# bensonlzl/spaced-kmer-sketching

Hardware: AMD Instinct MI355X
Metric: k-mers hashed/s + genome-pairs ANI/s at 1/2/4/8 MI355X; % HBM roofline (higher is better)
Workload: dtype u64; 1 GPU; config3: 1x3 Gb multi-contig genome per GPU, spaced seed w=31/k=21 (mask seed 0), FracMinHash 1/1000; builds_in_flight=3, genome_bytes=3000000024, windows_per_genome=2999036400, sketch_size=2998764, parallelism=genome-sharded x1

## Files before the change

### spaced-kmer-sketching_amd/csrc/build.cpp

```cpp
#include <cstdlib>
#include <numeric>
#include <utility>

#include "build_internal.hpp"

using namespace sks;

BuildKnobs sks::read_build_knobs() {
  static const bool scan_static = getenv("SKS_SCAN_STATIC") != nullptr;
  BuildKnobs k;
  k.no_fused_bottom = getenv("SKS_NO_FUSED_BOTTOM") != nullptr;
  k.no_fast_bottom = getenv("SKS_NO_FAST_BOTTOM") != nullptr;
  k.no_frac_fused = getenv("SKS_NO_FRAC_FUSED") != nullptr;
  k.scan_static = scan_static;
  return k;
}

int sks::validate_build(const char* fn, sks_ctx* c, const uint8_t* d_seq, uint64_t n_bytes, const uint64_t* seg_off,
                        uint32_t n_seg, int window, const uint64_t mask[2], const sks_policy* policy) {
  const std::string f(fn);
  if (!c || !mask || !policy || (!seg_off && n_seg)) return sks::fail(SKS_E_ARG, f + ": null argument");
  if (window < 1 || window > 64)
    return sks::fail(SKS_E_ARG, f + ": window must be in [1, 64] (MAX_KMER_LENGTH)");
  if (policy->kind != SKS_FRAC_MOD && policy->kind != SKS_BOTTOM_S)
// ... 29 lines not shown
  *out = {{}, arena.ptr(o_extra), arena.ptr(o_cnt), arena.ptr(o_cnt) + 2 * (m + 1)};
  sks::ScanParams& p = out->p;
  p.seq = d_seq;
  p.seg_begin = arena.ptr(o_beg);
  p.seg_end = arena.ptr(o_end);
  p.tile_prefix = arena.ptr(o_tiles);
  p.n_seg = g.m();
  p.n_tiles = g.n_tiles();
  p.w = S.w;
  p.mask_lo = S.mask_lo;
  p.mask_hi = S.mask_hi;
  p.kconst = S.kconst;
  p.low_mask = S.dt.low_mask;
  p.high_mask = S.dt.rot > 32 ? (uint32_t)((1ull << (S.dt.rot - 32)) - 1) : 0u;
  p.dinv = S.dt.dinv;
  p.dlim = S.dt.lim;
  p.seg_thresh = arena.ptr(list_mode ? o_cap : o_thr);
  p.out_key = reinterpret_cast<uint64_t*>(c->rec[0].ptr);
  p.seg_out_off = arena.ptr(o_off);
  p.seg_out_cap = arena.ptr(o_cap);
  p.seg_count = reinterpret_cast<unsigned long long*>(out->counters);
  p.seg_windows = reinterpret_cast<unsigned long long*>(out->counters + m + 1);
  if (list_mode) return SKS_OK;
  p.out_val = reinterpret_cast<uint64_t*>(c->rec[1].ptr);
  p.out_hi = reinterpret_cast<uint64_t*>(c->rec[2].ptr);
  p.tile_queue = S.knobs.scan_static ? nullptr : reinterpret_cast<unsigned long long*>(arena.ptr(o_queue));
  return SKS_OK;
}

namespace {

constexpr int kFastFallback = -1;
constexpr int kFastPostFallback = -2;

int make_single_set(const BuildState& S, uint64_t slots, SetPtr* one) {
  const uint64_t mask[2] = {S.mask_lo, S.mask_hi};
  return make_sketch_set(S.c->device, 1, S.w, mask, S.pol, {0}, {0}, {}, &slots, S.c->stream, MetaUpload::kNone, one);
}

template <class Post>
int run_single(const BuildState& S, const ScanMeta& meta, int mode, Post post, uint64_t h[6]) {
  sks_ctx* c = S.c;
  hipStream_t st = c->stream;
  hipError_t e = hipEventRecord(c->ev_s0, st);
  if (e == hipSuccess) e = sks::launch_scan(meta.p, mode, S.pol.flavour, false, c->device, st, c->grid_override);
  if (e == hipSuccess) e = hipEventRecord(c->ev_s1, st);
  if (e == hipSuccess) e = post();
// ... 43 lines not shown
  }, h));
  const uint64_t survivors = h[0], windows = h[2], size = h[4];
  if (survivors > cap || size == ~0ull || size == sks::kBottomOverflow || size > slots) return kFastFallback;
  scan_timings(c, seg.n_tiles(), survivors, tm);
  finish_single(S, tm, windows, size, one, out);
  return SKS_OK;
}

int build_frac_single(BuildState& S, const uint8_t* d_seq, const uint64_t* seg_off, uint64_t cap, int log_b,
                      sks_timings& tm, sks_sketch_set** out, uint64_t* survivors_out, uint64_t* windows_out) {
  sks_ctx* c = S.c;
  hipStream_t st = c->stream;
  const uint32_t bucket_cap = c->frac_bucket_cap
                                  ? std::min<uint32_t>(c->frac_bucket_cap, sks::frac_bucket_capacity())
                                  : sks::frac_bucket_capacity();
  const uint64_t slots = std::max<uint64_t>(cap, 1);
  SKS_HIP(c->rec[0].reserve(slots * sizeof(uint64_t)));
  SKS_HIP(c->buf[0].reserve(((uint64_t)bucket_cap << log_b) * sizeof(uint64_t)));
  SKS_HIP(c->fstate.reserve(sks::frac_state_bytes()));
  if (!c->fstate_clean) SKS_HIP(hipMemsetAsync(c->fstate.ptr, 0, sks::frac_state_bytes(), st));
  c->fstate_clean = false;
  ScanSegs seg;
  seg.push(seg_off[0], seg_off[1], ~0ull, cap);
  ScanMeta meta;
  SKS_TRY(scan_meta(S, d_seq, seg, false, {}, 2, &meta));
  SetPtr one;
  SKS_TRY(make_single_set(S, slots, &one));
  uint64_t h[6] = {0, 0, 0, 0, 0, 0};
  const int rc = run_single(S, meta, sks::kModeFrac, [&] {
    const hipError_t e = sks::launch_frac_fused(
        reinterpret_cast<uint64_t*>(c->rec[0].ptr), meta.counters, meta.p.seg_out_cap, slots, S.key_bits, S.runs,
        (uint32_t)log_b, bucket_cap, col(c, 0), reinterpret_cast<uint32_t*>(c->fstate.ptr), one->d_data(),
        one->d_sizes(), one->d_starts(), meta.results, st);
    if (e == hipSuccess) c->fstate_clean = true;
    return e;
  }, h);
  if (rc != SKS_OK) {
    c->fstate_clean = false;
    return rc;
  }
  const uint64_t survivors = h[0], windows = h[2], size = h[4], status = h[5];
  scan_timings(c, seg.n_tiles(), survivors, tm);
  *survivors_out = survivors;
  if (survivors > cap || size > survivors) return kFastFallback;
  if (status != 0) {
    *windows_out = windows;
    return kFastPostFallback;
  }
  finish_single(S, tm, windows, size, one, out);
  c->last_path = SKS_BUILD_PATH_FUSED;
  return SKS_OK;
}

struct Passes {
  std::vector<SegPlan> plan;
  std::vector<uint64_t> windows;
// ... 172 lines not shown
```

### spaced-kmer-sketching_amd/csrc/post.hip

```cpp
#include <hip/hip_runtime.h>

#include <algorithm>
#include <cstdio>
#include <cstring>
#include <rocprim/rocprim.hpp>
#include <rocprim/block/block_radix_sort.hpp>

#include "code_objects.hpp"
#include "device_mem.hpp"
#include "post.hpp"
#include "sks_hash.hpp"
#include "wave_prims.hpp"

namespace sks {

hipError_t Scratch::reserve(size_t n) {
  if (n <= bytes) return hipSuccess;
  const size_t grown = bytes + bytes / 2;
  if (ptr) {
    if (owner) {
      cache_release_after(ptr, bytes, *owner);
    } else {
      (void)hipDeviceSynchronize();
      (void)hipFree(ptr);
// ... 52 lines not shown
    return hipSuccess;
  }
  size_t need = 0;
  hipError_t e;
  if constexpr (PAIRS)
    e = rocprim::segmented_radix_sort_pairs(nullptr, need, keys_in, keys_out, vals_in, vals_out,
                                            (unsigned)total, (unsigned)n_seg, d_off, d_off + 1, 0,
                                            end_bit, s);
  else
    e = rocprim::segmented_radix_sort_keys(nullptr, need, keys_in, keys_out, (unsigned)total,
                                           (unsigned)n_seg, d_off, d_off + 1, 0, end_bit, s);
  if (e != hipSuccess) return e;
  if ((e = tmp.reserve(need)) != hipSuccess) return e;
  need = tmp.bytes;
  if constexpr (PAIRS)
    return rocprim::segmented_radix_sort_pairs(tmp.ptr, need, keys_in, keys_out, vals_in, vals_out,
                                               (unsigned)total, (unsigned)n_seg, d_off, d_off + 1,
                                               0, end_bit, s);
  else
    return rocprim::segmented_radix_sort_keys(tmp.ptr, need, keys_in, keys_out, (unsigned)total,
                                              (unsigned)n_seg, d_off, d_off + 1, 0, end_bit, s);
}

__device__ __forceinline__ uint64_t runs_pack(uint64_t x, const BitRuns& r) {
  x &= r.mask;
#pragma unroll
  for (int i = 0; i < 6; ++i) {
    const uint64_t mv = r.mv[i];
    if (mv) {
      const uint64_t t = x & mv;
      x = (x ^ t) | (t >> (1 << i));
    }
  }
  return x;
}

__device__ __forceinline__ uint64_t runs_expand(uint64_t x, const BitRuns& r) {
  const int width = __popcll(r.mask);
  if (width < 64) x &= (1ull << width) - 1;
#pragma unroll
  for (int i = 5; i >= 0; --i) {
    const uint64_t mv = r.mv[i];
    if (mv) x = (x & ~mv) | ((x << (1 << i)) & mv);
  }
  return x & r.mask;
}

template <bool PACK>
__global__ void k_compact(const uint64_t* __restrict__ src, uint64_t* __restrict__ dst,
                          const uint64_t* __restrict__ src_off, const uint64_t* __restrict__ dst_off,
                          const BitRuns runs, int tag_shift) {
  const uint32_t g = blockIdx.y;
  const uint64_t len = dst_off[g + 1] - dst_off[g];
  const uint64_t so = src_off[g], d0 = dst_off[g];
  const uint64_t tag = tag_shift >= 0 ? (uint64_t)g << tag_shift : 0;
  for (uint64_t i = (uint64_t)blockIdx.x * kB + threadIdx.x; i < len; i += (uint64_t)gridDim.x * kB)
    dst[d0 + i] = (PACK ? runs_pack(src[so + i], runs) : src[so + i]) | tag;
}

__global__ void k_bits_expand(uint64_t* __restrict__ keys, uint64_t n, const BitRuns runs) {
  for (uint64_t i = (uint64_t)blockIdx.x * kB + threadIdx.x; i < n; i += (uint64_t)gridDim.x * kB)
    keys[i] = runs_expand(keys[i], runs);
}

__global__ void k_flags(const uint64_t* __restrict__ keys, const uint64_t* __restrict__ keys2,
                        const uint64_t* __restrict__ off, uint32_t* __restrict__ flag) {
  const uint32_t g = blockIdx.y;
  const uint64_t b = off[g], e = off[g + 1];
  for (uint64_t i = b + (uint64_t)blockIdx.x * kB + threadIdx.x; i < e; i += (uint64_t)gridDim.x * kB) {
    bool first = (i == b) || keys[i] != keys[i - 1] || (keys2 && keys2[i] != keys2[i - 1]);
// ... 493 lines not shown
    lt_m |= (lt ? 1u : 0u) << j;
    eq_m |= (eq ? 1u : 0u) << j;
  }
  uint32_t eq_rank = block_excl_scan<kSelWaves>((uint32_t)__builtin_popcount(eq_m), wsum);
  __syncthreads();
  uint32_t keep_m = lt_m;
#pragma unroll
  for (uint32_t j = 0; j < ITEMS; ++j)
    if ((eq_m >> j) & 1u) keep_m |= (eq_rank++ < sel.kk ? 1u : 0u) << j;
  uint32_t pos = block_excl_scan<kSelWaves>((uint32_t)__builtin_popcount(keep_m), wsum);
  __syncthreads();
  uint64_t* skept = reinterpret_cast<uint64_t*>(smem);
#pragma unroll
  for (uint32_t j = 0; j < ITEMS; ++j)
    if ((keep_m >> j) & 1u) skept[pos++] = k[j];
  __syncthreads();
  for (uint32_t i = tid; i < (uint32_t)lim; i += kSelB) dst[i] = runs_expand(skept[i], runs);
}

constexpr int kFracB = 256;
constexpr int kFracWaves = kFracB / 64;
constexpr uint32_t kFracItems = 16;
constexpr uint32_t kFracCap = kFracB * kFracItems;
constexpr int kFracPartB = 1024;
constexpr uint32_t kFracPartTile = 1u << 14;
constexpr int kFracSubLog = 11;
constexpr uint32_t kFracSub = 1u << kFracSubLog;
constexpr uint32_t kFracSubPer = kFracSub / kFracB;
constexpr uint32_t kFracSubMax = 32;
constexpr uint32_t kFracMaxLogB = 14;
constexpr uint32_t kFracStateCounts = 1u << kFracMaxLogB;
constexpr uint32_t kFracStateStatus = 2u << kFracMaxLogB;

__global__ __launch_bounds__(kFracPartB) void k_frac_partition(const uint64_t* __restrict__ rec,
                                                               const uint64_t* __restrict__ seg_count,
                                                               const uint64_t* __restrict__ seg_cap,
                                                               const BitRuns runs, int shift, uint32_t n_buckets,
                                                               uint32_t bucket_cap, uint64_t* __restrict__ regions,
                                                               uint32_t* __restrict__ state) {
  extern __shared__ uint32_t s_cur[];
  const uint64_t n = seg_count[0];
  if (n > seg_cap[0]) return;
  const uint64_t rows = (n + kFracPartB - 1) / kFracPartB;
  const uint64_t share = (rows + gridDim.x - 1) / gridDim.x * kFracPartB;
  const uint64_t lo = min((uint64_t)blockIdx.x * share, n), hi = min(lo + share, n);
  if (lo >= hi) return;
  auto bucket_of = [&](uint64_t key) {
    const uint64_t top = shift < 64 ? key >> shift : 0ull;
    return (uint32_t)min(top, (uint64_t)(n_buckets - 1));
  };
  for (uint32_t b = threadIdx.x; b < n_buckets; b += kFracPartB) s_cur[b] = 0;
  __syncthreads();
#pragma unroll 4
  for (uint64_t i = lo + threadIdx.x; i < hi; i += kFracPartB) atomicAdd(&s_cur[bucket_of(runs_pack(rec[i], runs))], 1u);
  __syncthreads();
  for (uint32_t b = threadIdx.x; b < n_buckets; b += kFracPartB) {
    const uint32_t c = s_cur[b];
    if (c) s_cur[b] = atomicAdd(&state[b], c);
  }
  __syncthreads();
  bool over = false;
#pragma unroll 4
  for (uint64_t i = lo + threadIdx.x; i < hi; i += kFracPartB) {
    const uint64_t key = runs_pack(rec[i], runs);
    const uint32_t b = bucket_of(key);
    const uint32_t slot = atomicAdd(&s_cur[b], 1u);
    if (slot < bucket_cap) regions[(uint64_t)b * bucket_cap + slot] = key;
    else over = true;
  }
  if (over) atomicOr(&state[kFracStateStatus], (uint32_t)kFracStatusBucket);
}

template <uint32_t ITEMS>
__device__ __forceinline__ void frac_sort_body(uint64_t* __restrict__ reg, uint32_t n, uint32_t b,
                                               uint32_t* __restrict__ state, const BitRuns& runs, int shift,
                                               uint64_t* skeys, uint32_t* sbin, uint32_t* wsum, uint32_t* wmax) {
  const int tid = threadIdx.x;
  uint64_t k[ITEMS];
#pragma unroll
  for (uint32_t j = 0; j < ITEMS; ++j) {
    const uint32_t i = j * kFracB + tid;
    k[j] = i < n ? reg[i] : ~0ull;
  }
  const uint64_t low = shift >= 64 ? ~0ull : (1ull << shift) - 1;
  const int sub_shift = shift > kFracSubLog ? shift - kFracSubLog : 0;
  auto sub_of = [&](uint64_t key) { return (uint32_t)min((key & low) >> sub_shift, (uint64_t)(kFracSub - 1)); };
#pragma unroll
  for (uint32_t j = 0; j < ITEMS; ++j)
    if (j * kFracB + tid < n) atomicAdd(&sbin[sub_of(k[j])], 1u);
  __syncthreads();
  uint32_t cb[kFracSubPer], sum = 0, mx = 0;
#pragma unroll
  for (uint32_t q = 0; q < kFracSubPer; ++q) {
    cb[q] = sbin[tid * kFracSubPer + q];
// ... 48 lines not shown
  }
  __syncthreads();
  const uint64_t before = tid ? skeys[tid * ITEMS - 1] : 0ull;
  uint32_t first_m = 0;
#pragma unroll
  for (uint32_t j = 0; j < ITEMS; ++j) {
    const uint32_t i = tid * ITEMS + j;
    k[j] = skeys[i];
    const bool first = i < n && (i == 0 || k[j] != (j ? k[j - 1] : before));
    first_m |= (first ? 1u : 0u) << j;
  }
  uint32_t distinct;
  uint32_t pos = block_excl_scan<kFracWaves>((uint32_t)__builtin_popcount(first_m), wsum, &distinct);
  __syncthreads();
#pragma unroll
  for (uint32_t j = 0; j < ITEMS; ++j)
    if ((first_m >> j) & 1u) skeys[pos++] = k[j];
  __syncthreads();
  for (uint32_t i = tid; i < distinct; i += kFracB) reg[i] = runs_expand(skeys[i], runs);
  if (tid == 0) state[kFracStateCounts + b] = distinct;
}

__global__ __launch_bounds__(kFracB) void k_frac_sort_unique(uint64_t* __restrict__ regions,
                                                             uint32_t* __restrict__ state, const BitRuns runs,
                                                             int shift, uint32_t bucket_cap) {
  __shared__ uint64_t skeys[kFracCap];
  __shared__ uint32_t sbin[kFracSub];
  __shared__ uint32_t wsum[kFracWaves], wmax[kFracWaves];
  __shared__ uint32_t s_n;
  const uint32_t b = blockIdx.x;
  const int tid = threadIdx.x;
  uint32_t* counts = state + kFracStateCounts;
  if (tid == 0) {
    s_n = state[b];
    state[b] = 0;
  }
#pragma unroll
  for (uint32_t q = 0; q < kFracSubPer; ++q) sbin[tid * kFracSubPer + q] = 0;
  __syncthreads();
  const uint32_t n = s_n;
  if (n == 0 || n > bucket_cap) {
    if (tid == 0) {
      counts[b] = 0;
      if (n) atomicOr(&state[kFracStateStatus], (uint32_t)kFracStatusBucket);
    }
    return;
  }
  uint64_t* reg = regions + (uint64_t)b * bucket_cap;
  if (n <= 4 * kFracB) frac_sort_body<4>(reg, n, b, state, runs, shift, skeys, sbin, wsum, wmax);
  else if (n <= 8 * kFracB) frac_sort_body<8>(reg, n, b, state, runs, shift, skeys, sbin, wsum, wmax);
  else frac_sort_body<kFracItems>(reg, n, b, state, runs, shift, skeys, sbin, wsum, wmax);
}

__global__ __launch_bounds__(kFracB) void k_frac_gather(const uint64_t* __restrict__ regions,
                                                        uint32_t* __restrict__ state, uint32_t n_buckets,
                                                        uint32_t bucket_cap, uint64_t out_cap,
                                                        uint64_t* __restrict__ out, uint32_t* __restrict__ set_sizes,
// ... 45 lines not shown
                          uint64_t* vals_out, uint64_t total, const std::vector<uint64_t>& host_off,
                          const uint64_t* d_off, int end_bit, Scratch& tmp, hipStream_t s) {
  return sort_impl<true>(keys_in, keys_out, vals_in, vals_out, total, host_off, d_off, end_bit,
                         tmp, s);
}

hipError_t compact_regions(const uint64_t* src, uint64_t* dst, const uint64_t* d_src_off,
                           const uint64_t* d_dst_off, uint32_t n_seg, uint64_t max_len,
                           hipStream_t s, const BitRuns* pack, int tag_shift) {
  if (n_seg == 0 || max_len == 0) return hipSuccess;
  if (pack && pack->n)
    hipLaunchKernelGGL(k_compact<true>, dim3(grid_for(max_len), n_seg), dim3(kB), 0, s, src, dst,
                       d_src_off, d_dst_off, *pack, tag_shift);
  else
    hipLaunchKernelGGL(k_compact<false>, dim3(grid_for(max_len), n_seg), dim3(kB), 0, s, src, dst,
                       d_src_off, d_dst_off, BitRuns{}, tag_shift);
  return hipGetLastError();
}

hipError_t launch_seg_ids(uint64_t* out, const uint64_t* d_off, uint32_t n_seg, uint64_t max_len, hipStream_t s) {
  if (n_seg == 0 || max_len == 0) return hipSuccess;
  hipLaunchKernelGGL(k_seg_ids, dim3(grid_for(max_len), n_seg), dim3(kB), 0, s, out, d_off);
  return hipGetLastError();
}

BitRuns bit_runs(uint64_t mask) {
  BitRuns r;
  for (int b = 0; b < 64; ++b)
    if (((mask >> b) & 1) && (b == 0 || !((mask >> (b - 1)) & 1))) ++r.n;
  r.mask = mask;
  uint64_t m = mask, mk = ~m << 1;
  for (int i = 0; i < 6; ++i) {
    uint64_t mp = mk ^ (mk << 1);
    for (int sh = 2; sh < 64; sh <<= 1) mp ^= mp << sh;
    const uint64_t mv = mp & m;
    r.mv[i] = mv;
    m = (m ^ mv) | (mv >> (1 << i));
    mk &= ~mp;
  }
  return r;
}

hipError_t launch_bits_expand(uint64_t* keys, uint64_t n, const BitRuns& runs, hipStream_t s) {
  if (n == 0 || runs.n == 0) return hipSuccess;
  hipLaunchKernelGGL(k_bits_expand, dim3(grid_for(n)), dim3(kB), 0, s, keys, n, runs);
  return hipGetLastError();
}

hipError_t seg_unique_scan(const uint64_t* keys, const uint64_t* keys2, uint64_t total,
                           uint64_t max_len, const uint64_t* d_off, uint32_t n_seg, uint32_t* d_flag,
                           uint64_t* d_pos, uint64_t* d_uniq, Scratch& tmp, hipStream_t s) {
  if (n_seg == 0) return hipSuccess;
  hipError_t e;
  if (total) {
    hipLaunchKernelGGL(k_flags, dim3(grid_for(std::min<uint64_t>(max_len, 1ull << 24)), n_seg),
                       dim3(kB), 0, s, keys, keys2, d_off, d_flag);
    if ((e = hipGetLastError()) != hipSuccess) return e;
  }
  if ((e = hipMemsetAsync(d_flag + total, 0, sizeof(uint32_t), s)) != hipSuccess) return e;
  size_t need = 0;
  e = rocprim::exclusive_scan(nullptr, need, d_flag, d_pos, (uint64_t)0, (size_t)(total + 1),
                              rocprim::plus<uint64_t>(), s);
  if (e != hipSuccess) return e;
// ... 153 lines not shown
                               uint64_t* set_starts) {
  if (n_seg == 0) return hipSuccess;
  if (max_cnt > kFuseCap) return hipErrorInvalidValue;
  auto go = [&](auto kernel, size_t lds) -> hipError_t {
    const hipError_t a = hipFuncSetAttribute(reinterpret_cast<const void*>(kernel),
                                             hipFuncAttributeMaxDynamicSharedMemorySize, (int)lds);
    if (a != hipSuccess) return a;
    hipLaunchKernelGGL(kernel, dim3(n_seg), dim3(kSelB), lds, s, rec, d_src_off, d_cnt, d_retry_ok,
                       d_dst_off, s_param, key_bits, runs, kconst, out, d_res, d_cap, set_sizes, set_starts);
    return hipGetLastError();
  };
  if (max_cnt <= kSelB * 8)
    return flavour == 0 ? go(k_bottom_fused<0, 8>, fuse_lds<8>()) : go(k_bottom_fused<1, 8>, fuse_lds<8>());
  if (max_cnt <= kSelB * 12)
    return flavour == 0 ? go(k_bottom_fused<0, 12>, fuse_lds<12>())
                        : go(k_bottom_fused<1, 12>, fuse_lds<12>());
  return flavour == 0 ? go(k_bottom_fused<0, 16>, fuse_lds<16>()) : go(k_bottom_fused<1, 16>, fuse_lds<16>());
}

uint32_t frac_bucket_capacity() { return kFracCap; }
uint32_t frac_max_log_buckets() { return kFracMaxLogB; }
size_t frac_state_bytes() { return (size_t)(kFracStateStatus + 2) * sizeof(uint32_t); }

hipError_t launch_frac_fused(const uint64_t* rec, const uint64_t* d_cnt, const uint64_t* d_cap, uint64_t cap,
                             int key_bits, const BitRuns& runs, uint32_t log_b, uint32_t bucket_cap,
                             uint64_t* regions, uint32_t* state, uint64_t* out, uint32_t* set_sizes,
                             uint64_t* set_starts, uint64_t* d_res, hipStream_t s) {
  if (log_b > kFracMaxLogB || bucket_cap == 0 || bucket_cap > kFracCap || key_bits < 1 || key_bits > 64)
    return hipErrorInvalidValue;
  const uint32_t n_buckets = 1u << log_b;
  const int shift = key_bits > (int)log_b ? key_bits - (int)log_b : 0;
  const uint64_t tiles = (std::max<uint64_t>(cap, 1) + kFracPartTile - 1) / kFracPartTile;
  hipLaunchKernelGGL(k_frac_partition, dim3((unsigned)std::min<uint64_t>(tiles, 256)), dim3(kFracPartB),
                     n_buckets * sizeof(uint32_t), s, rec, d_cnt, d_cap, runs, shift, n_buckets, bucket_cap, regions,
                     state);
  hipLaunchKernelGGL(k_frac_sort_unique, dim3(n_buckets), dim3(kFracB), 0, s, regions, state, runs, shift,
                     bucket_cap);
  hipLaunchKernelGGL(k_frac_gather, dim3(n_buckets), dim3(kFracB), 0, s, regions, state, n_buckets, bucket_cap,
                     cap, out, set_sizes, set_starts, d_res);
  return hipGetLastError();
}

hipError_t launch_iota(uint64_t* out, uint64_t n, hipStream_t s) {
  if (n == 0) return hipSuccess;
  hipLaunchKernelGGL(k_iota, dim3(grid_for(n)), dim3(kB), 0, s, out, n);
  return hipGetLastError();
}

hipError_t launch_gather(const uint64_t* src, const uint64_t* idx, uint64_t n, uint64_t* out,
                         hipStream_t s) {
  if (n == 0) return hipSuccess;
  hipLaunchKernelGGL(k_gather, dim3(grid_for(n)), dim3(kB), 0, s, src, idx, n, out);
  return hipGetLastError();
}

hipError_t launch_interleave(const uint64_t* lo, const uint64_t* hi, uint64_t n, uint64_t* out,
                             hipStream_t s) {
  if (n == 0) return hipSuccess;
  hipLaunchKernelGGL(k_interleave, dim3(grid_for(n)), dim3(kB), 0, s, lo, hi, n, out);
  return hipGetLastError();
// ... 6 lines not shown
```

### spaced-kmer-sketching_amd/csrc/post.hpp

```cpp
#pragma once
#include <hip/hip_runtime.h>

#include <cstdint>
#include <vector>

#include "build_plan.hpp"
#include "device_mem.hpp"

namespace sks {

hipError_t seg_sort_keys(const uint64_t* keys_in, uint64_t* keys_out, uint64_t total,
                         const std::vector<uint64_t>& host_off, const uint64_t* d_off,
                         int end_bit, Scratch& tmp, hipStream_t s);
hipError_t seg_sort_pairs(const uint64_t* keys_in, uint64_t* keys_out, const uint64_t* vals_in,
                          uint64_t* vals_out, uint64_t total, const std::vector<uint64_t>& host_off,
                          const uint64_t* d_off, int end_bit, Scratch& tmp, hipStream_t s);

struct BitRuns {
  uint32_t n = 0;
  uint64_t mask = 0;
  uint64_t mv[6] = {0, 0, 0, 0, 0, 0};
};
BitRuns bit_runs(uint64_t mask);
hipError_t launch_bits_expand(uint64_t* keys, uint64_t n, const BitRuns& runs, hipStream_t s);
constexpr uint64_t kBottomOverflow = ~1ull;
uint32_t bottom_fused_capacity();
hipError_t launch_bottom_fused(uint64_t* rec, const uint64_t* d_src_off, const uint64_t* d_cnt,
                               const uint64_t* d_retry_ok, const uint64_t* d_dst_off,
                               uint32_t n_seg, uint64_t max_cnt, uint64_t s_param, int key_bits,
                               const BitRuns& runs, uint64_t kconst, int flavour, uint64_t* out,
                               uint64_t* d_res, hipStream_t s, const uint64_t* d_cap = nullptr,
                               uint32_t* set_sizes = nullptr, uint64_t* set_starts = nullptr);

constexpr uint64_t kFracStatusBucket = 1;
constexpr uint64_t kFracStatusCrowd = 2;
uint32_t frac_bucket_capacity();
uint32_t frac_max_log_buckets();
size_t frac_state_bytes();
hipError_t launch_frac_fused(const uint64_t* rec, const uint64_t* d_cnt, const uint64_t* d_cap, uint64_t cap,
                             int key_bits, const BitRuns& runs, uint32_t log_b, uint32_t bucket_cap,
                             uint64_t* regions, uint32_t* state, uint64_t* out, uint32_t* set_sizes,
                             uint64_t* set_starts, uint64_t* d_res, hipStream_t s);

hipError_t compact_regions(const uint64_t* src, uint64_t* dst, const uint64_t* d_src_off,
                           const uint64_t* d_dst_off, uint32_t n_seg, uint64_t max_len,
                           hipStream_t s, const BitRuns* pack = nullptr, int tag_shift = -1);
hipError_t launch_seg_ids(uint64_t* out, const uint64_t* d_off, uint32_t n_seg, uint64_t max_len, hipStream_t s);

hipError_t seg_unique_scan(const uint64_t* keys, const uint64_t* keys2, uint64_t total,
                           uint64_t max_len, const uint64_t* d_off, uint32_t n_seg, uint32_t* d_flag,
                           uint64_t* d_pos, uint64_t* d_uniq, Scratch& tmp, hipStream_t s);
hipError_t sort_unique_u64(const uint64_t* in, uint64_t n, uint64_t* out, uint64_t* n_out,
                           Scratch& tmp, hipStream_t s);
hipError_t sort_unique_u128(const uint64_t* in, uint64_t n, uint64_t* out, uint64_t* n_out,
                            Scratch& tmp, hipStream_t s);
hipError_t seg_unique_scatter(const uint64_t* vals, const uint64_t* vals2, uint64_t total,
                              uint64_t max_len, const uint64_t* d_off, uint32_t n_seg,
                              const uint32_t* d_flag,
                              const uint64_t* d_pos, const uint64_t* d_limit,
                              const uint64_t* d_dst_off, uint64_t* out, uint64_t* out2,
                              hipStream_t s, const BitRuns* expand = nullptr, uint64_t keep = ~0ull,
                              uint64_t keep2 = ~0ull);

hipError_t launch_synth(uint8_t* out, uint64_t n, uint64_t seed, uint64_t mut_seed,
                        uint64_t mut_thresh, uint64_t pos_offset, hipStream_t s);
// ... 19 lines not shown
```

### spaced-kmer-sketching_amd/csrc/scan.hip

```cpp
#include <hip/hip_runtime.h>

#include <cstdlib>

#include <cstdint>
#include <type_traits>

#include "code_objects.hpp"
#include "scan.hpp"
#include "sks_hash.hpp"

namespace sks {

namespace {

constexpr int kBlock = 256;
constexpr int kWPT = 16;
constexpr int kTile = kBlock * kWPT;
constexpr int kHaloWords = 4;
constexpr int kWords = kBlock + kHaloWords;
constexpr int kLoadVecs = (kWords * 16 + 16) / 16;
constexpr int kQCap = 2048;
#ifndef SKS_SCAN_QCAP
#define SKS_SCAN_QCAP 512
#endif
template <int MODE>
constexpr int qcap() { return MODE == kModeList ? kQCap : SKS_SCAN_QCAP; }
// ... 154 lines not shown

__device__ __forceinline__ uint32_t rev_pairs(uint32_t x) {
  uint32_t r = __builtin_bitreverse32(x);
  return ((r >> 1) & 0x55555555u) | ((r & 0x55555555u) << 1);
}


__device__ __forceinline__ unsigned long long wave_aggregated_inc(unsigned long long* counter) {
  const uint64_t act = __ballot(true);
  const uint32_t rank = __builtin_amdgcn_mbcnt_hi((uint32_t)(act >> 32),
                                                  __builtin_amdgcn_mbcnt_lo((uint32_t)act, 0u));
  unsigned long long base = 0;
  if (rank == 0) base = atomicAdd(counter, (unsigned long long)__popcll(act));
  const uint32_t lo = __builtin_amdgcn_readfirstlane((uint32_t)base);
  const uint32_t hi = __builtin_amdgcn_readfirstlane((uint32_t)(base >> 32));
  return (((unsigned long long)hi << 32) | lo) + rank;
}

template <int MODE>
struct Queue {
  uint64_t key[qcap<MODE>()];
  uint64_t val[MODE == kModeBottom ? qcap<MODE>() : 1];
  uint32_t n;
  unsigned long long base;
  unsigned long long wins;
};

template <int MODE>
__device__ __forceinline__ void emit(const ScanParams& p, Queue<MODE>& q, uint32_t seg,
                                     uint64_t key, uint64_t val) {
  uint32_t slot = atomicAdd(&q.n, 1u);
  if (slot < (uint32_t)qcap<MODE>()) {
    q.key[slot] = key;
    if constexpr (MODE == kModeBottom) q.val[slot] = val;
  } else {
    unsigned long long g = wave_aggregated_inc(&p.seg_count[seg]);
    if (g < p.seg_out_cap[seg]) {
      uint64_t o = p.seg_out_off[seg] + g;
      p.out_key[o] = key;
      if constexpr (MODE == kModeBottom) p.out_val[o] = val;
    }
  }
}

template <int MODE>
__device__ __forceinline__ void flush(const ScanParams& p, Queue<MODE>& q, uint32_t seg) {
  __syncthreads();
  if (threadIdx.x == 0 && q.wins) atomicAdd(&p.seg_windows[seg], q.wins);
  constexpr uint32_t cap = qcap<MODE>();
  uint32_t n = q.n < cap ? q.n : cap;
  if (n) {
    if (threadIdx.x == 0) q.base = atomicAdd(&p.seg_count[seg], (unsigned long long)n);
    __syncthreads();
    uint64_t base = q.base;
    uint64_t cap = p.seg_out_cap[seg];
    uint64_t off = p.seg_out_off[seg];
    for (uint32_t i = threadIdx.x; i < n; i += kBlock) {
      if (base + i < cap) {
        p.out_key[off + base + i] = q.key[i];
        if constexpr (MODE == kModeBottom) p.out_val[off + base + i] = q.val[i];
      }
    }
  }
  __syncthreads();
  if (threadIdx.x == 0) {
    q.n = 0;
    q.wins = 0;
  }
  __syncthreads();
}

__device__ __forceinline__ void add_windows(unsigned long long& wins, uint32_t cnt) {
  uint32_t v = cnt;
#pragma unroll
  for (int o = 32; o > 0; o >>= 1) v += __shfl_xor(v, o, 64);
  if ((threadIdx.x & 63) == 0 && v) atomicAdd(&wins, (unsigned long long)v);
}

template <int FLAVOUR>
__device__ __forceinline__ uint64_t fmh_narrow(const ScanParams& p, uint64_t c) {
  uint64_t h;
  if constexpr (FLAVOUR == 0) {
    h = hash_mix(c + kGolden32);
    h = hash_mix(h + kGolden32);
    h = hash_mix(h + (128 + kGolden32));
  } else {
    h = hash_bitset128<1>(c, 0);
  }
  return h ^ p.kconst;
}
// ... 37 lines not shown
__global__ __launch_bounds__(kBlock, (min_waves<MODE, PRE, FMIN>())) void scan_kernel(ScanParams p) {
  __shared__ uint32_t s_raw[kLoadVecs * 4];
  __shared__ uint32_t s_be[kWords + 2 + kBeOff];
  __shared__ uint32_t s_lc[kWords + 2];
  __shared__ uint32_t s_inv[kWords + 2];
  __shared__ Queue<MODE> q;
  __shared__ ulonglong2 s_cand[PRE ? (kBlock / 64) * kCandCap : 1];
  __shared__ uint32_t s_ctop[PRE ? kBlock / 64 : 1];

  __shared__ unsigned long long s_next;

  const int tid = threadIdx.x;
  const bool dyn = p.tile_queue != nullptr;
  uint64_t t_begin, t_end;
  if (dyn) {
    t_begin = (uint64_t)blockIdx.x * p.chunk;
    t_end = min(t_begin + p.chunk, p.n_tiles);
  } else {
    t_begin = (uint64_t)blockIdx.x * p.n_tiles / gridDim.x;
    t_end = (uint64_t)(blockIdx.x + 1) * p.n_tiles / gridDim.x;
  }
  if (tid == 0) {
    q.n = 0;
    q.wins = 0;
  }
  if (t_begin >= t_end) return;
  unsigned long long grab = 0;

  const int w = p.w;
  const uint32_t dshift = 2 * (32 - w);
  const uint64_t wmask_bits = (w >= 64) ? ~0ull : ((1ull << w) - 1);
  if (tid < kBeOff) s_be[tid] = 0;
  const uint32_t r = tid & 15;
  const uint32_t wbase = (uint32_t)(tid >> 4) * kWPT;
  const uint32_t of = 2 * r + 64 - dshift;
  const uint32_t qf = (of - 1) >> 5;
  const uint32_t sF = 32 * qf + 32 - of;
  const uint32_t sR = 2 * r;
  const uint32_t* const fb = s_be + (kBeOff - 2) + wbase + qf;
  const uint32_t* const rb = s_lc + wbase;

  uint32_t seg_lo = 0, seg_hi = p.n_seg;
  while (seg_lo + 1 < seg_hi) {
    uint32_t mid = (seg_lo + seg_hi) >> 1;
    if (p.tile_prefix[mid] <= t_begin) seg_lo = mid; else seg_hi = mid;
  }
// ... 514 lines not shown
```

### spaced-kmer-sketching_amd/csrc/scan.hpp

```cpp
#pragma once
#include <hip/hip_runtime.h>

#include <cstdint>

namespace sks {

constexpr int kModeFrac = 0;
constexpr int kModeBottom = 1;
constexpr int kModeList = 2;

struct ScanParams {
  const uint8_t* seq;
  const uint64_t* seg_begin;
  const uint64_t* seg_end;
  const uint64_t* tile_prefix;
  uint32_t n_seg;
  uint64_t n_tiles;
  int w;
  uint64_t mask_lo, mask_hi;
  uint64_t kconst;
  uint32_t low_mask, high_mask;
  uint64_t dinv, dlim;
  const uint64_t* seg_thresh;
  uint64_t* out_key;
  uint64_t* out_val;
  uint64_t* out_hi;
  const uint64_t* seg_out_off;
  const uint64_t* seg_out_cap;
  unsigned long long* seg_count;
  unsigned long long* seg_windows;
  unsigned long long* tile_queue;
  uint32_t chunk;
};

uint64_t scan_tiles_for(uint64_t seg_bytes);
hipError_t launch_scan(const ScanParams& p, int mode, int flavour, bool wide, int device,
                       hipStream_t stream, int grid_override);

}
```

Before: 785.9 billion k-mers/s.

## Fuse FracMinHash bucket partitioning into the scan kernel's queue flush

The separate k_frac_partition kernel, which re-read all scan survivors from the record buffer and scattered them into per-bucket regions, is removed. The scan kernel now packs each surviving key and atomically places it into its bucket region when it flushes its LDS queue, reading a bucket descriptor uploaded in scan metadata via constant address space. The sort kernel now checks the overflow condition itself. This drops one kernel launch and a full reread of the survivor array, at the cost of per-key global atomics on bucket cursors inside the scan and extra register and code pressure in the hot scan kernel.

```diff
diff --git a/spaced-kmer-sketching_amd/csrc/bit_runs.hpp b/spaced-kmer-sketching_amd/csrc/bit_runs.hpp
--- /dev/null
+++ b/spaced-kmer-sketching_amd/csrc/bit_runs.hpp
@@ -0,0 +1,97 @@
+#pragma once
+#include <cstddef>
+#include <cstdint>
+
+#if defined(__HIPCC__)
+#define SKS_HD __host__ __device__ __forceinline__
+#define SKS_UNROLL _Pragma("unroll")
+#define SKS_NO_UNROLL _Pragma("unroll 1")
+#else
+#define SKS_HD inline
+#define SKS_UNROLL
+#define SKS_NO_UNROLL
+#endif
+
+namespace sks {
+
+struct BitRuns {
+  uint32_t n = 0;
+  uint64_t mask = 0;
+  uint64_t mv[6] = {0, 0, 0, 0, 0, 0};
+};
+
+inline BitRuns bit_runs(uint64_t mask) {
+  BitRuns r;
+  for (int b = 0; b < 64; ++b)
+    if (((mask >> b) & 1) && (b == 0 || !((mask >> (b - 1)) & 1))) ++r.n;
+  r.mask = mask;
+  uint64_t m = mask, mk = ~m << 1;
+  for (int i = 0; i < 6; ++i) {
+    uint64_t mp = mk ^ (mk << 1);
+    for (int sh = 2; sh < 64; sh <<= 1) mp ^= mp << sh;
+    const uint64_t mv = mp & m;
+    r.mv[i] = mv;
+    m = (m ^ mv) | (mv >> (1 << i));
+    mk &= ~mp;
+  }
+  return r;
+}
+
+SKS_HD uint64_t runs_pack(uint64_t x, const BitRuns& r) {
+  x &= r.mask;
+SKS_UNROLL
+  for (int i = 0; i < 6; ++i) {
+    const uint64_t mv = r.mv[i];
+    if (mv) {
+      const uint64_t t = x & mv;
+      x = (x ^ t) | (t >> (1 << i));
+    }
+  }
+  return x;
+}
+
+template <class Words>
+SKS_HD uint64_t runs_pack_rolled(uint64_t x, Words words) {
+  x &= words[0];
+SKS_NO_UNROLL
+  for (uint32_t i = 0; i < 6; ++i) {
+    const uint64_t t = x & words[1 + i];
+    x = (x ^ t) | (t >> (1u << i));
+  }
+  return x;
+}
+static_assert(offsetof(BitRuns, mv) == offsetof(BitRuns, mask) + sizeof(uint64_t), "runs_pack_rolled's layout");
+
+SKS_HD uint64_t runs_expand(uint64_t x, const BitRuns& r) {
+  const int width = __builtin_popcountll(r.mask);
+  if (width < 64) x &= (1ull << width) - 1;
+SKS_UNROLL
+  for (int i = 5; i >= 0; --i) {
+    const uint64_t mv = r.mv[i];
+    if (mv) x = (x & ~mv) | ((x << (1 << i)) & mv);
+  }
+  return x & r.mask;
+}
+
+SKS_HD int frac_bucket_shift(int key_bits, uint32_t log_b) {
+  return key_bits > (int)log_b ? key_bits - (int)log_b : 0;
+}
+SKS_HD uint32_t frac_bucket_of(uint64_t packed_key, int shift, uint32_t n_buckets) {
+  const uint64_t top = shift < 64 ? packed_key >> shift : 0ull;
+  return (uint32_t)(top < (uint64_t)(n_buckets - 1) ? top : (uint64_t)(n_buckets - 1));
+}
+
+struct FracBuckets {
+  BitRuns runs;
+  int32_t shift;
+  uint32_t n_buckets;
+  uint32_t bucket_cap;
+  uint32_t status_bit;
+  uint64_t* regions;
+  uint32_t* cursors;
+  uint32_t* status;
+};
+static_assert(sizeof(FracBuckets) % sizeof(uint64_t) == 0, "uploaded as 64-bit words");
+static_assert(offsetof(FracBuckets, runs) == 0, "the scan reads the descriptor by its offsets");
+
+}
diff --git a/spaced-kmer-sketching_amd/csrc/build.cpp b/spaced-kmer-sketching_amd/csrc/build.cpp
--- a/spaced-kmer-sketching_amd/csrc/build.cpp
+++ b/spaced-kmer-sketching_amd/csrc/build.cpp
@@ -1,4 +1,5 @@
 #include <cstdlib>
+#include <cstring>
 #include <numeric>
 #include <utility>
 
@@ -75,7 +76,8 @@
   p.seg_count = reinterpret_cast<unsigned long long*>(out->counters);
   p.seg_windows = reinterpret_cast<unsigned long long*>(out->counters + m + 1);
   if (list_mode) return SKS_OK;
-  p.out_val = reinterpret_cast<uint64_t*>(c->rec[1].ptr);
+  if (S.pol.kind == SKS_FRAC_MOD && !S.wide) p.buckets = nullptr;
+  else p.out_val = reinterpret_cast<uint64_t*>(c->rec[1].ptr);
   p.out_hi = reinterpret_cast<uint64_t*>(c->rec[2].ptr);
   p.tile_queue = S.knobs.scan_static ? nullptr : reinterpret_cast<unsigned long long*>(arena.ptr(o_queue));
   return SKS_OK;
@@ -165,16 +167,20 @@
   c->fstate_clean = false;
   ScanSegs seg;
   seg.push(seg_off[0], seg_off[1], ~0ull, cap);
+  uint32_t* const state = reinterpret_cast<uint32_t*>(c->fstate.ptr);
+  const sks::FracBuckets desc = sks::frac_buckets(S.key_bits, S.runs, (uint32_t)log_b, bucket_cap, col(c, 0), state);
+  std::vector<uint64_t> desc_words(sizeof(desc) / sizeof(uint64_t));
+  memcpy(desc_words.data(), &desc, sizeof(desc));
   ScanMeta meta;
-  SKS_TRY(scan_meta(S, d_seq, seg, false, {}, 2, &meta));
+  SKS_TRY(scan_meta(S, d_seq, seg, false, desc_words, 2, &meta));
+  meta.p.buckets = reinterpret_cast<const sks::FracBuckets*>(meta.extra);
   SetPtr one;
   SKS_TRY(make_single_set(S, slots, &one));
   uint64_t h[6] = {0, 0, 0, 0, 0, 0};
   const int rc = run_single(S, meta, sks::kModeFrac, [&] {
-    const hipError_t e = sks::launch_frac_fused(
-        reinterpret_cast<uint64_t*>(c->rec[0].ptr), meta.counters, meta.p.seg_out_cap, slots, S.key_bits, S.runs,
-        (uint32_t)log_b, bucket_cap, col(c, 0), reinterpret_cast<uint32_t*>(c->fstate.ptr), one->d_data(),
-        one->d_sizes(), one->d_starts(), meta.results, st);
+    const hipError_t e = sks::launch_frac_fused(meta.counters, meta.p.seg_out_cap, slots, S.key_bits, S.runs,
+                                                (uint32_t)log_b, bucket_cap, col(c, 0), state, one->d_data(),
+                                                one->d_sizes(), one->d_starts(), meta.results, st);
     if (e == hipSuccess) c->fstate_clean = true;
     return e;
   }, h);
diff --git a/spaced-kmer-sketching_amd/csrc/post.hip b/spaced-kmer-sketching_amd/csrc/post.hip
--- a/spaced-kmer-sketching_amd/csrc/post.hip
+++ b/spaced-kmer-sketching_amd/csrc/post.hip
@@ -98,30 +98,6 @@
                                               (unsigned)n_seg, d_off, d_off + 1, 0, end_bit, s);
 }
 
-__device__ __forceinline__ uint64_t runs_pack(uint64_t x, const BitRuns& r) {
-  x &= r.mask;
-#pragma unroll
-  for (int i = 0; i < 6; ++i) {
-    const uint64_t mv = r.mv[i];
-    if (mv) {
-      const uint64_t t = x & mv;
-      x = (x ^ t) | (t >> (1 << i));
-    }
-  }
-  return x;
-}
-
-__device__ __forceinline__ uint64_t runs_expand(uint64_t x, const BitRuns& r) {
-  const int width = __popcll(r.mask);
-  if (width < 64) x &= (1ull << width) - 1;
-#pragma unroll
-  for (int i = 5; i >= 0; --i) {
-    const uint64_t mv = r.mv[i];
-    if (mv) x = (x & ~mv) | ((x << (1 << i)) & mv);
-  }
-  return x & r.mask;
-}
-
 template <bool PACK>
 __global__ void k_compact(const uint64_t* __restrict__ src, uint64_t* __restrict__ dst,
                           const uint64_t* __restrict__ src_off, const uint64_t* __restrict__ dst_off,
@@ -661,8 +637,6 @@
 constexpr int kFracWaves = kFracB / 64;
 constexpr uint32_t kFracItems = 16;
 constexpr uint32_t kFracCap = kFracB * kFracItems;
-constexpr int kFracPartB = 1024;
-constexpr uint32_t kFracPartTile = 1u << 14;
 constexpr int kFracSubLog = 11;
 constexpr uint32_t kFracSub = 1u << kFracSubLog;
 constexpr uint32_t kFracSubPer = kFracSub / kFracB;
@@ -670,45 +644,6 @@
 constexpr uint32_t kFracMaxLogB = 14;
 constexpr uint32_t kFracStateCounts = 1u << kFracMaxLogB;
 constexpr uint32_t kFracStateStatus = 2u << kFracMaxLogB;
-
-__global__ __launch_bounds__(kFracPartB) void k_frac_partition(const uint64_t* __restrict__ rec,
-                                                               const uint64_t* __restrict__ seg_count,
-                                                               const uint64_t* __restrict__ seg_cap,
-                                                               const BitRuns runs, int shift, uint32_t n_buckets,
-                                                               uint32_t bucket_cap, uint64_t* __restrict__ regions,
-                                                               uint32_t* __restrict__ state) {
-  extern __shared__ uint32_t s_cur[];
-  const uint64_t n = seg_count[0];
-  if (n > seg_cap[0]) return;
-  const uint64_t rows = (n + kFracPartB - 1) / kFracPartB;
-  const uint64_t share = (rows + gridDim.x - 1) / gridDim.x * kFracPartB;
-  const uint64_t lo = min((uint64_t)blockIdx.x * share, n), hi = min(lo + share, n);
-  if (lo >= hi) return;
-  auto bucket_of = [&](uint64_t key) {
-    const uint64_t top = shift < 64 ? key >> shift : 0ull;
-    return (uint32_t)min(top, (uint64_t)(n_buckets - 1));
-  };
-  for (uint32_t b = threadIdx.x; b < n_buckets; b += kFracPartB) s_cur[b] = 0;
-  __syncthreads();
-#pragma unroll 4
-  for (uint64_t i = lo + threadIdx.x; i < hi; i += kFracPartB) atomicAdd(&s_cur[bucket_of(runs_pack(rec[i], runs))], 1u);
-  __syncthreads();
-  for (uint32_t b = threadIdx.x; b < n_buckets; b += kFracPartB) {
-    const uint32_t c = s_cur[b];
-    if (c) s_cur[b] = atomicAdd(&state[b], c);
-  }
-  __syncthreads();
-  bool over = false;
-#pragma unroll 4
-  for (uint64_t i = lo + threadIdx.x; i < hi; i += kFracPartB) {
-    const uint64_t key = runs_pack(rec[i], runs);
-    const uint32_t b = bucket_of(key);
-    const uint32_t slot = atomicAdd(&s_cur[b], 1u);
-    if (slot < bucket_cap) regions[(uint64_t)b * bucket_cap + slot] = key;
-    else over = true;
-  }
-  if (over) atomicOr(&state[kFracStateStatus], (uint32_t)kFracStatusBucket);
-}
 
 template <uint32_t ITEMS>
 __device__ __forceinline__ void frac_sort_body(uint64_t* __restrict__ reg, uint32_t n, uint32_t b,
@@ -803,7 +738,9 @@
 }
 
 __global__ __launch_bounds__(kFracB) void k_frac_sort_unique(uint64_t* __restrict__ regions,
-                                                             uint32_t* __restrict__ state, const BitRuns runs,
+                                                             uint32_t* __restrict__ state,
+                                                             const uint64_t* __restrict__ seg_count,
+                                                             const uint64_t* __restrict__ seg_cap, const BitRuns runs,
                                                              int shift, uint32_t bucket_cap) {
   __shared__ uint64_t skeys[kFracCap];
   __shared__ uint32_t sbin[kFracSub];
@@ -813,7 +750,7 @@
   const int tid = threadIdx.x;
   uint32_t* counts = state + kFracStateCounts;
   if (tid == 0) {
-    s_n = state[b];
+    s_n = seg_count[0] > seg_cap[0] ? 0u : state[b];
     state[b] = 0;
   }
 #pragma unroll
@@ -905,23 +842,6 @@
   if (n_seg == 0 || max_len == 0) return hipSuccess;
   hipLaunchKernelGGL(k_seg_ids, dim3(grid_for(max_len), n_seg), dim3(kB), 0, s, out, d_off);
   return hipGetLastError();
-}
-
-BitRuns bit_runs(uint64_t mask) {
-  BitRuns r;
-  for (int b = 0; b < 64; ++b)
-    if (((mask >> b) & 1) && (b == 0 || !((mask >> (b - 1)) & 1))) ++r.n;
-  r.mask = mask;
-  uint64_t m = mask, mk = ~m << 1;
-  for (int i = 0; i < 6; ++i) {
-    uint64_t mp = mk ^ (mk << 1);
-    for (int sh = 2; sh < 64; sh <<= 1) mp ^= mp << sh;
-    const uint64_t mv = mp & m;
-    r.mv[i] = mv;
-    m = (m ^ mv) | (mv >> (1 << i));
-    mk &= ~mp;
-  }
-  return r;
 }
 
 hipError_t launch_bits_expand(uint64_t* keys, uint64_t n, const BitRuns& runs, hipStream_t s) {
@@ -1121,20 +1041,30 @@
 uint32_t frac_max_log_buckets() { return kFracMaxLogB; }
 size_t frac_state_bytes() { return (size_t)(kFracStateStatus + 2) * sizeof(uint32_t); }
 
-hipError_t launch_frac_fused(const uint64_t* rec, const uint64_t* d_cnt, const uint64_t* d_cap, uint64_t cap,
-                             int key_bits, const BitRuns& runs, uint32_t log_b, uint32_t bucket_cap,
-                             uint64_t* regions, uint32_t* state, uint64_t* out, uint32_t* set_sizes,
-                             uint64_t* set_starts, uint64_t* d_res, hipStream_t s) {
+FracBuckets frac_buckets(int key_bits, const BitRuns& runs, uint32_t log_b, uint32_t bucket_cap, uint64_t* regions,
+                         uint32_t* state) {
+  FracBuckets d;
+  d.runs = runs;
+  d.shift = frac_bucket_shift(key_bits, log_b);
+  d.n_buckets = 1u << log_b;
+  d.bucket_cap = bucket_cap;
+  d.status_bit = (uint32_t)kFracStatusBucket;
+  d.regions = regions;
+  d.cursors = state;
+  d.status = state + kFracStateStatus;
+  return d;
+}
+
+hipError_t launch_frac_fused(const uint64_t* d_cnt, const uint64_t* d_cap, uint64_t cap, int key_bits,
+                             const BitRuns& runs, uint32_t log_b, uint32_t bucket_cap, uint64_t* regions,
+                             uint32_t* state, uint64_t* out, uint32_t* set_sizes, uint64_t* set_starts,
+                             uint64_t* d_res, hipStream_t s) {
   if (log_b > kFracMaxLogB || bucket_cap == 0 || bucket_cap > kFracCap || key_bits < 1 || key_bits > 64)
     return hipErrorInvalidValue;
   const uint32_t n_buckets = 1u << log_b;
-  const int shift = key_bits > (int)log_b ? key_bits - (int)log_b : 0;
-  const uint64_t tiles = (std::max<uint64_t>(cap, 1) + kFracPartTile - 1) / kFracPartTile;
-  hipLaunchKernelGGL(k_frac_partition, dim3((unsigned)std::min<uint64_t>(tiles, 256)), dim3(kFracPartB),
-                     n_buckets * sizeof(uint32_t), s, rec, d_cnt, d_cap, runs, shift, n_buckets, bucket_cap, regions,
-                     state);
-  hipLaunchKernelGGL(k_frac_sort_unique, dim3(n_buckets), dim3(kFracB), 0, s, regions, state, runs, shift,
-                     bucket_cap);
+  const int shift = frac_bucket_shift(key_bits, log_b);
+  hipLaunchKernelGGL(k_frac_sort_unique, dim3(n_buckets), dim3(kFracB), 0, s, regions, state, d_cnt, d_cap, runs,
+                     shift, bucket_cap);
   hipLaunchKernelGGL(k_frac_gather, dim3(n_buckets), dim3(kFracB), 0, s, regions, state, n_buckets, bucket_cap,
                      cap, out, set_sizes, set_starts, d_res);
   return hipGetLastError();
diff --git a/spaced-kmer-sketching_amd/csrc/post.hpp b/spaced-kmer-sketching_amd/csrc/post.hpp
--- a/spaced-kmer-sketching_amd/csrc/post.hpp
+++ b/spaced-kmer-sketching_amd/csrc/post.hpp
@@ -4,6 +4,7 @@
 #include <cstdint>
 #include <vector>
 
+#include "bit_runs.hpp"
 #include "build_plan.hpp"
 #include "device_mem.hpp"
 
@@ -16,12 +17,6 @@
                           uint64_t* vals_out, uint64_t total, const std::vector<uint64_t>& host_off,
                           const uint64_t* d_off, int end_bit, Scratch& tmp, hipStream_t s);
 
-struct BitRuns {
-  uint32_t n = 0;
-  uint64_t mask = 0;
-  uint64_t mv[6] = {0, 0, 0, 0, 0, 0};
-};
-BitRuns bit_runs(uint64_t mask);
 hipError_t launch_bits_expand(uint64_t* keys, uint64_t n, const BitRuns& runs, hipStream_t s);
 constexpr uint64_t kBottomOverflow = ~1ull;
 uint32_t bottom_fused_capacity();
@@ -37,10 +32,12 @@
 uint32_t frac_bucket_capacity();
 uint32_t frac_max_log_buckets();
 size_t frac_state_bytes();
-hipError_t launch_frac_fused(const uint64_t* rec, const uint64_t* d_cnt, const uint64_t* d_cap, uint64_t cap,
-                             int key_bits, const BitRuns& runs, uint32_t log_b, uint32_t bucket_cap,
-                             uint64_t* regions, uint32_t* state, uint64_t* out, uint32_t* set_sizes,
-                             uint64_t* set_starts, uint64_t* d_res, hipStream_t s);
+FracBuckets frac_buckets(int key_bits, const BitRuns& runs, uint32_t log_b, uint32_t bucket_cap, uint64_t* regions,
+                         uint32_t* state);
+hipError_t launch_frac_fused(const uint64_t* d_cnt, const uint64_t* d_cap, uint64_t cap, int key_bits,
+                             const BitRuns& runs, uint32_t log_b, uint32_t bucket_cap, uint64_t* regions,
+                             uint32_t* state, uint64_t* out, uint32_t* set_sizes, uint64_t* set_starts,
+                             uint64_t* d_res, hipStream_t s);
 
 hipError_t compact_regions(const uint64_t* src, uint64_t* dst, const uint64_t* d_src_off,
                            const uint64_t* d_dst_off, uint32_t n_seg, uint64_t max_len,
diff --git a/spaced-kmer-sketching_amd/csrc/scan.hip b/spaced-kmer-sketching_amd/csrc/scan.hip
--- a/spaced-kmer-sketching_amd/csrc/scan.hip
+++ b/spaced-kmer-sketching_amd/csrc/scan.hip
@@ -2,6 +2,7 @@
 
 #include <cstdlib>
 
+#include <cstddef>
 #include <cstdint>
 #include <type_traits>
 
@@ -202,15 +203,61 @@
   uint64_t key[qcap<MODE>()];
   uint64_t val[MODE == kModeBottom ? qcap<MODE>() : 1];
   uint32_t n;
+  uint32_t over;
   unsigned long long base;
   unsigned long long wins;
 };
+
+typedef const __attribute__((address_space(4))) uint8_t* ConstBytes;
+template <class T>
+__device__ __forceinline__ T desc_field(ConstBytes desc, size_t offset) {
+  return *reinterpret_cast<const __attribute__((address_space(4))) T*>(desc + offset);
+}
+__device__ __forceinline__ bool place_in_bucket(const FracBuckets* buckets, uint64_t key) {
+  uint64_t at = (uint64_t)(uintptr_t)buckets;
+  asm volatile("" : "+s"(at));
+  const ConstBytes d = reinterpret_cast<ConstBytes>((uintptr_t)at);
+  typedef const __attribute__((address_space(4))) uint64_t* ConstWords;
+  const uint64_t packed =
+      runs_pack_rolled(key, reinterpret_cast<ConstWords>(d + offsetof(FracBuckets, runs) + offsetof(BitRuns, mask)));
+  asm volatile("" : "+s"(at));
+  const ConstBytes e = reinterpret_cast<ConstBytes>((uintptr_t)at);
+  const uint32_t b = frac_bucket_of(packed, desc_field<int32_t>(e, offsetof(FracBuckets, shift)),
+                                    desc_field<uint32_t>(e, offsetof(FracBuckets, n_buckets)));
+  const uint32_t slot = atomicAdd(desc_field<uint32_t*>(e, offsetof(FracBuckets, cursors)) + b, 1u);
+  const uint32_t bucket_cap = desc_field<uint32_t>(e, offsetof(FracBuckets, bucket_cap));
+  if (slot < bucket_cap) {
+    desc_field<uint64_t*>(e, offsetof(FracBuckets, regions))[(uint64_t)b * bucket_cap + slot] = packed;
+    return false;
+  }
+  return true;
+}
+__device__ __forceinline__ void raise_bucket_status(const FracBuckets* buckets) {
+  const ConstBytes d = reinterpret_cast<ConstBytes>((uintptr_t)buckets);
+  atomicOr(desc_field<uint32_t*>(d, offsetof(FracBuckets, status)),
+           desc_field<uint32_t>(d, offsetof(FracBuckets, status_bit)));
+}
+__device__ __forceinline__ void place_direct(const FracBuckets* buckets, uint64_t key) {
+  if (place_in_bucket(buckets, key)) {
+    const uint64_t act = __ballot(true);
+    const uint32_t rank = __builtin_amdgcn_mbcnt_hi((uint32_t)(act >> 32), __builtin_amdgcn_mbcnt_lo((uint32_t)act, 0u));
+    if (rank == 0) raise_bucket_status(buckets);
+  }
+}
+typedef const __attribute__((address_space(3))) uint64_t* LdsKeys;
+__device__ __forceinline__ bool place_queue(const FracBuckets* buckets, LdsKeys keys, uint32_t n, uint64_t room) {
+  bool over = false;
+#pragma unroll 1
+  for (uint32_t i = threadIdx.x; i < n; i += kBlock)
+    if (i < room) over |= place_in_bucket(buckets, keys[i]);
+  return over;
+}
 
 template <int MODE>
 __device__ __forceinline__ void emit(const ScanParams& p, Queue<MODE>& q, uint32_t seg,
                                      uint64_t key, uint64_t val) {
   uint32_t slot = atomicAdd(&q.n, 1u);
-  if (slot < (uint32_t)qcap<MODE>()) {
+  if (__builtin_expect(slot < (uint32_t)qcap<MODE>(), 1)) {
     q.key[slot] = key;
     if constexpr (MODE == kModeBottom) q.val[slot] = val;
   } else {
@@ -219,6 +266,9 @@
       uint64_t o = p.seg_out_off[seg] + g;
       p.out_key[o] = key;
       if constexpr (MODE == kModeBottom) p.out_val[o] = val;
+      if constexpr (MODE == kModeFrac) {
+        if (__builtin_expect(p.buckets != nullptr, 0)) place_direct(p.buckets, key);
+      }
     }
   }
 }
@@ -241,11 +291,23 @@
         if constexpr (MODE == kModeBottom) p.out_val[off + base + i] = q.val[i];
       }
     }
+    if constexpr (MODE == kModeFrac) {
+      if (p.buckets != nullptr) {
+        const LdsKeys keys = (LdsKeys)(uintptr_t)(__attribute__((address_space(3))) void*)q.key;
+        if (place_queue(p.buckets, keys, n, base < cap ? cap - base : 0)) q.over = 1;
+      }
+    }
   }
   __syncthreads();
   if (threadIdx.x == 0) {
     q.n = 0;
     q.wins = 0;
+    if constexpr (MODE == kModeFrac) {
+      if (p.buckets != nullptr && q.over) {
+        q.over = 0;
+        raise_bucket_status(p.buckets);
+      }
+    }
   }
   __syncthreads();
 }
@@ -329,6 +391,7 @@
   }
   if (tid == 0) {
     q.n = 0;
+    q.over = 0;
     q.wins = 0;
   }
   if (t_begin >= t_end) return;
diff --git a/spaced-kmer-sketching_amd/csrc/scan.hpp b/spaced-kmer-sketching_amd/csrc/scan.hpp
--- a/spaced-kmer-sketching_amd/csrc/scan.hpp
+++ b/spaced-kmer-sketching_amd/csrc/scan.hpp
@@ -2,6 +2,8 @@
 #include <hip/hip_runtime.h>
 
 #include <cstdint>
+
+#include "bit_runs.hpp"
 
 namespace sks {
 
@@ -23,7 +25,10 @@
   uint64_t dinv, dlim;
   const uint64_t* seg_thresh;
   uint64_t* out_key;
-  uint64_t* out_val;
+  union {
+    uint64_t* out_val;
+    const FracBuckets* buckets;
+  };
   uint64_t* out_hi;
   const uint64_t* seg_out_off;
   const uint64_t* seg_out_cap;
@@ -32,6 +37,7 @@
   unsigned long long* tile_queue;
   uint32_t chunk;
 };
+static_assert(sizeof(ScanParams) == 184, "ScanParams grew");
 
 uint64_t scan_tiles_for(uint64_t seg_bytes);
 hipError_t launch_scan(const ScanParams& p, int mode, int flavour, bool wide, int device,
```

Result: no change. 785.6 billion k-mers/s (-0.0%).
